# triSYCL/path_tracer

Measured on AMD Instinct MI355X. Metric: Msamples/s (W x H x spp / s) at 1080p 1024spp, higher is better.
Workload: dtype f32; 1 GPU; cornell: Cornell-style 7 box + 1 xy_rect + diffuse light, 1920x1080, 1024 spp, depth 50, seed = pixel linear id; hittables=8, mode=parity, frame_at_1_gpu=1920x1080

## Files before the change

path_tracer_amd/csrc/pt_device.hpp:

```cpp
#pragma once
#include <hip/hip_runtime.h>
#include <stdint.h>

#include "pt_math.hpp"

#ifdef PT_STAMPS
extern __device__ unsigned long long g_stamps[8];
#endif
#ifdef PT_STAMPS_TRI
extern __device__ unsigned long long g_tri[16];
#endif
#ifdef PT_STAMPS_RUNS
extern __device__ unsigned long long g_runs[16];
#endif
#ifdef PT_STAMPS_WALK
extern __device__ unsigned long long g_walk[8];
__device__ __forceinline__ unsigned long long* walk_ctr() { __shared__ unsigned long long c[8]; return c; }
#define PT_WALK_COUNT(i, v) do { const unsigned long long v_ = (unsigned long long)(v); if ((threadIdx.x & 63) == 0) atomicAdd(&walk_ctr()[i], v_); } while (0)
#else
#define PT_WALK_COUNT(i, v) do { } while (0)
#endif

namespace ptd {

// ... 820 lines not shown
  const cst_i4p lists = (cst_i4p)(cblob + lists_off);
  i4 cur = lists[0];
  for (int q = 0; q < q_static; ++q) {
    const i4 nxt = lists[q + 1];
    sphere_list_entry<false, K>(recs, cur, goff, 0.0f, c, h, accept_at);
    cur = nxt;
  }
  for (int q = 0; q < q_moving; ++q) {
    const i4 nxt = lists[q_static + q + 1];
    sphere_list_entry<true, K>(recs, cur, goff, frac, c, h, accept_at);
    cur = nxt;
  }
#ifdef PT_STAMPS_WALK
  const unsigned long long walk_t0 = __builtin_amdgcn_s_memtime();
  __builtin_amdgcn_sched_barrier(0);
#endif
  if constexpr (GRID == 1) { if (walk) sphere_grid_walk(recs, recs + w_cell, recs + w_cand, wg0, wg1, frac, goff, c, h, accept_at); }
  if constexpr (GRID == 2) {
    if (walk) {
      unsigned long long* slot;
      unsigned int* q;
      if constexpr (TRIPOOL) { slot = tri_slots() + (threadIdx.x & ~63); q = (unsigned int*)(tri_queue() + (threadIdx.x >> 6) * PT_TRI_QUEUE); }
      else { slot = sphere_slots() + (threadIdx.x & ~63); q = sphere_queue() + (threadIdx.x >> 6) * PT_SQ_CAP; }
      sphere_grid_walk_queued(recs, recs + w_cell, recs + w_cand, wg0, wg1, frac, (flags & 2) != 0, goff, c, h, slot, q, accept_at);
    }
  }
#ifdef PT_STAMPS_WALK
  asm volatile("" ::"v"(h.closest), "v"(h.hit));
  __builtin_amdgcn_sched_barrier(0);
  if (GRID && walk) { PT_WALK_COUNT(0, __builtin_amdgcn_s_memtime() - walk_t0); PT_WALK_COUNT(1, 1); }
#endif
}

template <bool FILTER, typename P>
__device__ __forceinline__ unsigned long long slab_chunk_pass(P xrecs, P slrecs, cst_f4p srecs, int cn, float bmax, const RayCtx& c, V3 om, V3 op, float& kdone,
                                                HitState& h) {
  const float none = as_f(PT_KEY_NONE);
  auto ku = [](float k) { return (unsigned int)as_i(k); };
  float k1 = none, k2 = none, k3 = none;
  typedef float f16v __attribute__((ext_vector_type(16)));
  typedef const __attribute__((address_space(4))) f16v* cst_f16p;
  const cst_f16p pairs = (cst_f16p)srecs;
  auto entry = [&](float lx, float ly, float lz, float hx, float hy, float hz, int j) {
    const float ax = __builtin_fmaf(lx, c.yx, om.x), bx = __builtin_fmaf(hx, c.yx, op.x);
    const float ay = __builtin_fmaf(ly, c.yy, om.y), by = __builtin_fmaf(hy, c.yy, op.y);
    const float az = __builtin_fmaf(lz, c.yz, om.z), bz = __builtin_fmaf(hz, c.yz, op.z);
    const float tn = __builtin_fmaxf(__builtin_fmaxf(__builtin_fminf(ax, bx), __builtin_fminf(ay, by)), __builtin_fminf(az, bz));
    const float tf = __builtin_fminf(__builtin_fminf(__builtin_fmaxf(ax, bx), __builtin_fmaxf(ay, by)), __builtin_fmaxf(az, bz));
    const float L = __builtin_fmaxf(tn, PT_TMIN);
    float key;
    asm("v_bfi_b32 %0, 15, %1, %2" : "=v"(key) : "s"(j), "v"(L));
    bool cand = L <= tf;
    if (FILTER) cand = cand & (ku(key) > ku(kdone));
    const float kk = cand ? key : none;
    asm("v_med3_u32 %0, %1, %0, %2" : "+v"(k3) : "v"(k2), "v"(kk));
    asm("v_med3_u32 %0, %1, %0, %2" : "+v"(k2) : "v"(k1), "v"(kk));
    asm("v_min_u32_e32 %0, %0, %1" : "+v"(k1) : "v"(kk));
  };
  for (int j = 0; j < cn; j += 2) {
    const f16v e = pairs[j >> 1];
    entry(e[0], e[1], e[2], e[4], e[5], e[6], j);
    entry(e[8], e[9], e[10], e[12], e[13], e[14], j + 1);
  }
  k1 = c.live ? k1 : none;
  k3 = c.live ? k3 : none;
  const unsigned long long had3 = __builtin_amdgcn_ballot_w64(ku(k3) != PT_KEY_NONE);
  unsigned long long vote;
#pragma unroll 1
  do {
    {
      bool inside = (ku(k1) ^ (unsigned int)as_i(PT_TMIN)) < 16u;
#ifdef PT_NO_POOL_PROOF
      inside = false;
#endif
      if (__builtin_amdgcn_ballot_w64(inside)) {
        const int offs = (as_i(k1) & 15) * 2;
        const f4 S0 = slrecs[offs], S1 = slrecs[offs + 1];
        const float e = 0x1p-20f, tlo = PT_TMIN * (1.0f - 0x1p-20f);
        auto ends = [&](float o, float y, float lo, float hi, float& lw, float& us, float& ws) {
          const float a = (lo - o) * y, b = (hi - o) * y;
          lw = __builtin_fminf(a, b);
          const float up = __builtin_fmaxf(a, b);
          const float S = __builtin_fmaf(__builtin_fabsf(o), 0x1.7p-21f, 0x1.dp-22f * bmax);
          const float w = __builtin_fmaf(__builtin_fabsf(y), S, up);
          us = __builtin_fmaf(__builtin_fabsf(up), -e, up);
          ws = __builtin_fmaf(__builtin_fabsf(w), e, w);
          return __builtin_fmaf(__builtin_fabsf(up), e, up) < PT_TMIN;
        };
        float lwx, lwy, lwz, usx, usy, usz, wsx, wsy, wsz;
        const bool ownx = ends(c.r.o.x, c.yx, S0.x, S1.x, lwx, usx, wsx);
        const bool owny = ends(c.r.o.y, c.yy, S0.y, S1.y, lwy, usy, wsy);
        const bool ownz = ends(c.r.o.z, c.yz, S0.z, S1.z, lwz, usz, wsz);
        const float lwm = __builtin_fmaxf(__builtin_fmaxf(lwx, lwy), lwz);
        const bool near_behind = __builtin_fmaf(__builtin_fabsf(lwm), e, lwm) < PT_TMIN;
        const bool kx = ownx & (usy > wsx) & (usz > wsx);
        const bool ky = owny & (usx > wsy) & (usz > wsy);
        const bool kz = ownz & (usx > wsz) & (usy > wsz);
        const bool gone = inside & near_behind & (kx | ky | kz);
        kdone = gone ? k1 : kdone;
        k1 = gone ? k2 : k1; k2 = gone ? k3 : k2; k3 = gone ? none : k3;
      }
    }
    asm("v_cmp_le_f32_e64 %0, %1, %2" : "=s"(vote) : "v"(as_i(k1) & ~15), "v"(h.closest));
    const bool active = __builtin_amdgcn_inverse_ballot_w64(vote);
#ifdef PT_STAMPS_POOL
    {
      const unsigned long long busy = __builtin_amdgcn_ballot_w64(active);
      if (vote != 0 && (threadIdx.x & 63) == 0) {
        atomicAdd(&g_stamps[5], 1ull);
        atomicAdd(&g_stamps[7], (unsigned long long)__builtin_popcountll(busy));
        if (FILTER) atomicAdd(&g_stamps[6], 1ull);
      }
    }
#endif
    if (active) {
      const int offl = (as_i(k1) & 15) * 2;
      const f4 X0 = xrecs[offl], X1 = xrecs[offl + 1];
      const unsigned long long exec_now = __builtin_amdgcn_ballot_w64(true);
      int hit_base = as_i(X0.w);
      const bool holder_later = ((h.hit >= 0) & (hit_off(h.hit) > hit_off(hit_base))) && hit_kind(h.hit) != DK_SPHERE;
      float cl = holder_later ? as_f(as_i(h.closest) - 1) : h.closest;
      int holder;
      asm("v_mov_b32_e32 %0, %1" : "=v"(holder) : "v"(h.hit));
      box_cmpx(X0, X1, c, exec_now, hit_base, cl, h.hit);
      asm("v_cmp_ne_u32_e32 vcc, %[hit], %[holder]\n\t"
          "v_mov_b32_e32 %[kd], %[k1]\n\t"
          "v_mov_b32_e32 %[k1], %[k2]\n\t"
          "v_cndmask_b32_e32 %[closest], %[closest], %[cl], vcc\n\t"
          "v_mov_b32_e32 %[k2], %[k3]\n\t"
          "v_mov_b32_e32 %[k3], %[none]"
          : [kd] "+v"(kdone), [k1] "+v"(k1), [k2] "+v"(k2), [k3] "+v"(k3), [closest] "+v"(h.closest)
          : [hit] "v"(h.hit), [holder] "v"(holder), [cl] "v"(cl), [none] "v"(none)
          : "vcc");
    }
  } while (vote != 0);
  return had3 & __builtin_amdgcn_ballot_w64(ku(k1) == PT_KEY_NONE);
}

template <typename P>
__device__ __forceinline__ void slab_pool(P blob, cst_f4p cblob, int pool_off, int n, float bmax, const RayCtx& c, HitState& h) {
  const float kP = 0x1.2p-21f;
  const float bP = 0x1.cp-22f * bmax;
  const V3 pp = mk(__builtin_fmaf(__builtin_fabsf(c.r.o.x), kP, bP), __builtin_fmaf(__builtin_fabsf(c.r.o.y), kP, bP),
                   __builtin_fmaf(__builtin_fabsf(c.r.o.z), kP, bP));
  const V3 yv = mk(c.yx, c.yy, c.yz);
  const V3 om = (mk(0.0f, 0.0f, 0.0f) - (c.r.o + pp)) * yv, op = (mk(0.0f, 0.0f, 0.0f) - (c.r.o - pp)) * yv;
#ifdef PT_STAMPS_POOL
  if ((threadIdx.x & 63) == 0) atomicAdd(&g_stamps[4], 1ull);
#endif
  for (int base = 0; base < n; base += 16) {
    const int cn = n - base < 16 ? n - base : 16;
    const P xrecs = blob + pool_off + 2 * (n + (n & 1)) + 2 * base;
    const cst_f4p srecs = cblob + pool_off + 2 * base;
    const P slrecs = blob + pool_off + 2 * base;
    float kdone = 0.0f;
    unsigned long long more = slab_chunk_pass<false>(xrecs, slrecs, srecs, cn, bmax, c, om, op, kdone, h);
    while (more) {
      if (!__builtin_amdgcn_inverse_ballot_w64(more)) kdone = as_f(PT_KEY_NONE);
      more = slab_chunk_pass<true>(xrecs, slrecs, srecs, cn, bmax, c, om, op, kdone, h);
    }
  }
}

#ifdef PT_STAMPS_TRI
#define PT_TRI_COUNT(i, v) do { const unsigned long long v_ = (unsigned long long)(v); if ((threadIdx.x & 63) == 0) atomicAdd(&g_tri[i], v_); } while (0)
#else
#define PT_TRI_COUNT(i, v) do { } while (0)
#endif
#define PT_TRI_WAVE_BITS(m) (__builtin_popcountll(__builtin_amdgcn_ballot_w64(((m) & 1u) != 0)) + __builtin_popcountll(__builtin_amdgcn_ballot_w64(((m) & 2u) != 0)) + \
                             __builtin_popcountll(__builtin_amdgcn_ballot_w64(((m) & 4u) != 0)) + __builtin_popcountll(__builtin_amdgcn_ballot_w64(((m) & 8u) != 0)))

__device__ __forceinline__ unsigned int gdword(glb_f4p pool, unsigned int base_f4, unsigned int i) { return ((const __attribute__((address_space(1))) unsigned int*)(pool + base_f4))[i]; }
__device__ __forceinline__ unsigned int gdword_stream(glb_f4p pool, unsigned int base_f4, unsigned int i) {
#ifdef PT_NT_LOADS
  return __builtin_nontemporal_load(((const __attribute__((address_space(1))) unsigned int*)(pool + base_f4)) + i);
#else
  return gdword(pool, base_f4, i);
#endif
}
__device__ __forceinline__ unsigned int sdword(glb_f4p pool, unsigned int base_f4, unsigned int i) {
  return ((const __attribute__((address_space(4))) unsigned int*)(unsigned long long)(pool + base_f4))[i];
}

typedef short short2_t __attribute__((ext_vector_type(2)));
#ifndef PT_BAND_PER
#define PT_BAND_PER 2
#endif
#define PT_TRI_BQUEUE (64 + 64 * PT_BAND_PER)
__device__ __forceinline__ f4* tri_bqueue() { __shared__ f4 s[4 * PT_TRI_BQUEUE]; return s; }
__device__ __forceinline__ int* tri_bqueue_idx() { __shared__ int s[4 * PT_TRI_BQUEUE]; return s; }
__device__ __forceinline__ unsigned long long tri_key(float t, int off) {
  return ((unsigned long long)(unsigned int)as_i(t) << 32) | (unsigned long long)(0xffffffffu - (unsigned int)off);
// ... 701 lines not shown
      if (IMG) { if (acc) { h.u = bu; h.v = bv; } }
    }
  }
}

__device__ __forceinline__ int record_size(int kind) {
  return kind == DK_SPHERE ? SZ_SPHERE : kind == DK_RECT ? SZ_RECT : (kind == DK_TRI || kind == DK_TRI_B) ? SZ_TRI : kind == DK_BOX ? SZ_BOX : SZ_MEDIUM;
}

template <bool IMG, bool BADOUEL = false, int GRID = 1, bool TRIPOOL = false, bool RECTBOX = false, bool DEFER = false, typename P>
__device__ __forceinline__ void hit_world_range(P blob, cst_f4p cblob, int ri0, int ri1, const RayCtx& c, bool fast, uint32_t& rng, HitState& h, const f4* pool = nullptr,
                                                TriDefer* dfr = nullptr, const TriPrimCtx* pc = nullptr) {
  for (int ri = ri0; ri < ri1; ++ri) {
#ifdef PT_STAMPS_RUNS
    const unsigned long long run_t0 = __builtin_amdgcn_s_memtime();
    __builtin_amdgcn_sched_barrier(0);
    struct RunStamp { unsigned long long t0; int ri; const HitState* h; __device__ ~RunStamp() { asm volatile("" ::"v"(h->closest), "v"(h->hit)); __builtin_amdgcn_sched_barrier(0);
      if ((threadIdx.x & 63) == 0) atomicAdd(&g_runs[ri < 15 ? ri : 15], __builtin_amdgcn_s_memtime() - t0); } } run_stamp{run_t0, ri, &h};
#endif
    f4 runf = cblob[ri];
    const int off = as_i(runf.y), kind = as_i(runf.x);
    if (!RECTBOX && (kind & DK_ABSORBED)) continue;
#ifdef PT_ABLATE_TAIL
    if (ri > 0) continue;
#endif
    if constexpr (RECTBOX) {
      static_assert(!IMG, "scenes of rects and boxes only have no image texture that tracks u, v");
      const f4 aux = cblob[off - 1];
      int span = fast ? as_i(aux.y) : 0;
#ifdef __HIP_DEVICE_COMPILE__
      asm volatile("" : "+s"(span));
#endif
      if (span != 0) {
        slab_pool(blob, cblob, as_i(aux.z), as_i(aux.w), aux.x, c, h);
        ri += span - 1;
      }
      hit_records_rectbox(blob + off, kind, span != 0 ? 0 : as_i(runf.z), off, c, fast, h);
    } else {
    if constexpr (!IMG) {
      if (fast && (kind == DK_RECT || kind == DK_BOX)) {
        const f4 aux = cblob[off - 1];
        if (as_i(aux.y) != 0) {
          slab_pool(blob, cblob, as_i(aux.z), as_i(aux.w), aux.x, c, h);
          ri += as_i(aux.y) - 1;
          continue;
        }
      }
    }
    hit_records<IMG, 1, 1, true, BADOUEL, GRID, TRIPOOL, RECTBOX, DEFER>(blob + off, cblob, kind, as_i(runf.z), off, c, fast, rng, h, (glb_f4p)pool, dfr, pc);
    }
  }
}
template <bool IMG, bool BADOUEL = false, int GRID = 1, bool TRIPOOL = false, bool RECTBOX = false, typename P>
__device__ __forceinline__ void hit_world(P blob, cst_f4p cblob, int n_runs, const RayCtx& c, bool fast, uint32_t& rng, HitState& h, const f4* pool = nullptr,
                                          const TriPrimCtx* pc = nullptr) {
  hit_begin(h);
  hit_world_range<IMG, BADOUEL, GRID, TRIPOOL, RECTBOX, false>(blob, cblob, 0, n_runs, c, fast, rng, h, pool, nullptr, pc);
}

__device__ __forceinline__ bool wave_all_regular(const RayCtx& c, bool live) {
  return __builtin_amdgcn_ballot_w64(live && !c.reg) == 0;
}

struct CoopScene {
  int n_runs;
  int coop_prefix;
};

__device__ __forceinline__ int nth_set_bit(unsigned long long m, int n) {
  for (int k = 0; k < n; ++k) m &= m - 1;
  return __builtin_ctzll(m);
}

__device__ __forceinline__ float shfl_f(float v, int src) { return __shfl(v, src, 64); }
__device__ __forceinline__ int shfl_i(int v, int src) { return __shfl(v, src, 64); }

// ... 360 lines not shown
```

path_tracer_amd/csrc/pt_flatten.hpp:

```cpp
#pragma once
#include <algorithm>
#include <cmath>
#include <cstdint>
#include <cstring>
#include <string>
#include <vector>

#include "../../include/pt_render.h"
#include "pt_tripool.hpp"

namespace ptf {

struct F4 {
  float x, y, z, w;
};
static_assert(sizeof(F4) == 16);

inline float as_f(int32_t i) { float f; std::memcpy(&f, &i, 4); return f; }

enum { DK_SPHERE = 0, DK_RECT = 1, DK_TRI = 2, DK_BOX = 3, DK_MEDIUM = 4, DK_TRI_B = 5 ,
       DK_ABSORBED = 8  };
enum { kHitOffBits = 25, kHitSideShift = 25, kHitKindShift = 28 };

struct PoolSegment { uint64_t at_f4; std::vector<uint32_t> dwords; };
struct PoolLayout {
  std::vector<PoolSegment> segments;
  uint64_t size_f4 = 0;
  uint32_t put(std::vector<uint32_t>&& v, int spare_f4) {
    const uint64_t at = size_f4;
    size_f4 += (v.size() + 3) / 4 + (uint64_t)spare_f4;
    segments.push_back(PoolSegment{at, std::move(v)});
    return (uint32_t)at;
  }
  void assemble(F4* out) const {
    std::memset((void*)out, 0, (size_t)size_f4 * 16);
    for (const PoolSegment& sg : segments) if (!sg.dwords.empty()) std::memcpy((void*)(out + sg.at_f4), sg.dwords.data(), sg.dwords.size() * 4);
  }
};
struct Flat {
  std::vector<F4> blob;
  std::vector<F4> mats;
  PoolLayout pool;
  int32_t n_runs = 0;
  bool has_image = false;
  bool has_medium = false;
  bool coop_ok = true;
  int32_t coop_prefix = 0;
  bool fast_ok = true;
  bool has_badouel = false;
  int grid_spheres = 0;
  int pooled = 0;
  int tri_pooled = 0;
  double tri_cells_per_triangle = 0;
  int tri_wide = 0, tri_maps = 0;
  long long tri_map_entries[3] = {0, 0, 0};
  int tri_map_res[3] = {0, 0, 0};
  int absorbed_spheres = 0;
  int tri_pool_runs = 0;
  int tri_pool_run = -1, tri_pool_hdr = 0, tri_pool_goff = 0, tri_pool_count = 0;
};

inline int device_kind(int32_t k) {
  switch (k) {
    case PT_HIT_SPHERE: return DK_SPHERE;
    case PT_HIT_XY_RECT: case PT_HIT_XZ_RECT: case PT_HIT_YZ_RECT: return DK_RECT;
    case PT_HIT_TRIANGLE: return DK_TRI;
    case PT_HIT_BOX: return DK_BOX;
    case PT_HIT_CONSTANT_MEDIUM: return DK_MEDIUM;
    default: return -1;
  }
}

inline int device_kind(const PtHittable& h) {
  if (h.kind == PT_HIT_TRIANGLE && h.strategy == PT_TRI_BADOUEL) return DK_TRI_B;
  return device_kind(h.kind);
}

inline int record_size(int dk) {
  switch (dk) { case DK_SPHERE: return 3; case DK_RECT: return 2; case DK_TRI: case DK_TRI_B: return 3; case DK_BOX: return 2; default: return 4; }
}

inline int validate(const PtSceneDesc* sc, std::string& err) {
  if (!sc) { err = "scene description is NULL"; return PT_ERR_INVALID_ARG; }
  if (sc->n_hittables < 0 || sc->n_materials < 0 || sc->n_textures < 0) { err = "negative table size"; return PT_ERR_INVALID_ARG; }
// ... 205 lines not shown
  for (uint32_t i : order) bandv.insert(bandv.end(), &tp.band_q[4 * (size_t)i], &tp.band_q[4 * (size_t)i] + 4);
  const uint32_t band = pool.put(std::move(bandv), 260);
  std::vector<uint32_t> readyv;
  readyv.reserve(12 * ntri);
  for (uint32_t i : order) for (int k = 0; k < 12; k++) readyv.push_back(bits(tp.band_ready[12 * (size_t)i + (size_t)k]));
  const uint32_t ready = pool.put(std::move(readyv), 192);
  const uint32_t cell_first = pool.put(std::move(tp.cell_first), 2);
  const uint32_t cell_cand = pool.put(std::move(tp.cell_cand), 20);
  uint32_t mfirst[kTriPoolMaxMaps] = {0, 0, 0}, mcand[kTriPoolMaxMaps] = {0, 0, 0};
  const int n_maps = std::min((int)tp.maps.size(), (int)kTriPoolMaxMaps);
  for (int k = 0; k < n_maps; k++) {
    TriDirMap& dm = tp.maps[(size_t)k];
    mfirst[k] = pool.put(std::move(dm.first), 2);
    mcand[k] = pool.put(std::move(dm.cand), 200);
  }
  const int32_t hdr = (int32_t)b.size();
  b.push_back({tp.origin[0], tp.origin[1], tp.origin[2], tp.inv_cell});
  b.push_back({as_f(tp.n[0]), as_f(tp.n[1]), as_f(tp.n[2]), tp.cell});
  b.push_back({tp.centre[0], tp.centre[1], tp.centre[2], tp.R});
  b.push_back({tp.rlimit2, tp.kappa, as_f((int32_t)ntri), as_f(n_maps)});
  b.push_back({as_f((int32_t)cell_first), as_f((int32_t)cell_cand), as_f((int32_t)tri_sorted), as_f((int32_t)band)});
  b.push_back({0.0f, tp.kq, tp.p_per_L, tp.kt});
  b.push_back({tp.ball_abs, tp.kr_a, tp.kr_b, tp.ea});
  b.push_back({tp.cq_lo[0], tp.cq_lo[1], tp.cq_lo[2], tp.eps_c});
  b.push_back({tp.cq_step[0], tp.cq_step[1], tp.cq_step[2], tp.eps_n});
  for (int k = 0; k < kTriPoolMaxMaps; k++) {
    if (k < n_maps) b.push_back({as_f(tp.maps[(size_t)k].R), tp.maps[(size_t)k].rho_max, as_f((int32_t)mfirst[k]), as_f((int32_t)mcand[k])});
    else b.push_back({as_f(0), -1.0f, as_f(0), as_f(0)});
  }
  b.push_back({as_f((int32_t)ready), 0.0f, 0.0f, 0.0f});
  return hdr;
}

inline int flatten(const PtSceneDesc* sc, Flat& out, std::string& err, bool allow_grid = true, int box_cull = 1, GridTuning tune = GridTuning(),
                   bool allow_tri_pool = true, TriPoolTuning tri_tune = TriPoolTuning(), bool sphere_merge = true) {
  int rc = validate(sc, err);
  if (rc) return rc;
  out = Flat();
  out.mats.reserve((size_t)sc->n_materials * 4);
  for (int i = 0; i < sc->n_materials; i++) {
    const PtMaterial& m = sc->materials[i];
    F4 M0{as_f(m.kind), as_f(PT_TEX_SOLID), m.param, 1.0f}, M1{m.color[0], m.color[1], m.color[2], as_f(1)},
        M2{0, 0, 0, as_f(1)}, M3{as_f(0), 0, 0, 0};
    if (m.kind == PT_MAT_LAMBERTIAN || m.kind == PT_MAT_LIGHTSOURCE || m.kind == PT_MAT_ISOTROPIC) {
      const PtTexture& t = sc->textures[m.texture];
      M0.y = as_f(t.kind);
      M0.w = t.freq;
      M1 = {t.color0[0], t.color0[1], t.color0[2], as_f((int32_t)t.width)};
      M2 = {t.color1[0], t.color1[1], t.color1[2], as_f((int32_t)t.height)};
      M3.x = as_f((int32_t)t.offset);
      if (t.kind == PT_TEX_IMAGE) out.has_image = true;
    }
    out.mats.push_back(M0); out.mats.push_back(M1); out.mats.push_back(M2); out.mats.push_back(M3);
  }
  struct Run { int kind, first, count; };
  std::vector<Run> runs;
  for (int i = 0; i < sc->n_hittables; i++) {
    int dk = device_kind(sc->hittables[i]);
    if (dk == DK_TRI_B) out.has_badouel = true;
    if (runs.empty() || runs.back().kind != dk) runs.push_back({dk, i, 0});
    runs.back().count++;
  }
  for (int i = 0; i < sc->n_hittables; i++) {
    const PtHittable& h = sc->hittables[i];
    bool rectish = h.kind == PT_HIT_XY_RECT || h.kind == PT_HIT_XZ_RECT || h.kind == PT_HIT_YZ_RECT || h.kind == PT_HIT_BOX ||
                   (h.kind == PT_HIT_CONSTANT_MEDIUM && h.boundary_kind == PT_HIT_BOX);
    if (!rectish) continue;
    int nf = (h.kind == PT_HIT_BOX || h.kind == PT_HIT_CONSTANT_MEDIUM) ? 6 : 5;
    for (int k = 0; k < nf; k++)
      if (!(std::fabs(h.f[k]) <= 1.152921504606846976e18f)) out.fast_ok = false;
    if (nf == 5) { if (!(h.f[0] <= h.f[1] && h.f[2] <= h.f[3])) out.fast_ok = false; }
// ... 46 lines not shown
  }
  struct Patch { size_t ri; std::vector<std::pair<size_t, size_t>> ranges; };
  std::vector<Patch> patches;
  for (size_t ri = 0; ri < runs.size(); ri++) {
    const Run& run = runs[ri];
    if (run.kind == DK_SPHERE) {
      std::vector<int32_t> codes;
      for (size_t k = 0; k < foreign_of[ri].size(); k++) codes.push_back(-(int32_t)(1 + k));
      Patch pt{ri, {}};
      out.grid_spheres += put_sphere_run_aux(b, &sc->hittables[run.first], run.count, allow_grid, tune, &codes, &pt.ranges);
      if (!codes.empty()) patches.push_back(std::move(pt));
      if (absorbed_by[ri] >= 0) { int32_t fl; std::memcpy(&fl, &b.back().w, 4); b.back().w = as_f(fl | 8); }
    }
    if (run.kind == DK_BOX || run.kind == DK_RECT) {
      const bool prev_rectish = ri > 0 && (runs[ri - 1].kind == DK_BOX || runs[ri - 1].kind == DK_RECT);
      int span = 0, n = 0, n_box = 0;
      if (!prev_rectish) {
        size_t rj = ri;
        while (rj < runs.size() && (runs[rj].kind == DK_BOX || runs[rj].kind == DK_RECT)) {
          n += runs[rj].count;
          if (runs[rj].kind == DK_BOX) n_box += runs[rj].count;
          rj++;
        }
        span = (int)(rj - ri);
      }
      const bool pool = box_cull && out.fast_ok && span > 0 && (box_cull == 2 ? n >= 2 : 88 * n_box - 7 * (n - n_box) > 200);
      float bmax = 0.0f;
      int32_t pool_off = 0;
      if (pool) {
        pool_off = (int32_t)b.size();
        pool_first = run.first;
        pool_at = b.size();
        const int ns = n + (n & 1);
        b.resize(b.size() + 2 * (size_t)ns + 2 * (size_t)n);
        pool_x = pool_at + 2 * (size_t)ns;
        if (ns > n) { const float q = std::nanf(""); b[pool_at + 2 * n] = {q, q, q, 0}; b[pool_at + 2 * n + 1] = {q, q, q, 0}; }
        const float ninf = -INFINITY;
        for (int e = 0; e < n; e++) {
          const PtHittable& h = sc->hittables[run.first + e];
          const float* f = h.f;
          F4 lo, hi, xhi;
          if (h.kind == PT_HIT_BOX) { lo = {f[0], f[1], f[2], 0}; hi = {f[3], f[4], f[5], 0}; xhi = hi; }
          else if (h.kind == PT_HIT_XY_RECT) { lo = {f[0], f[2], f[4], 0}; hi = {f[1], f[3], f[4], 0}; xhi = {f[1], f[3], ninf, 0}; }
          else if (h.kind == PT_HIT_XZ_RECT) { lo = {f[0], f[4], f[2], 0}; hi = {f[1], f[4], f[3], 0}; xhi = {f[1], ninf, f[3], 0}; }
          else { lo = {f[4], f[0], f[2], 0}; hi = {f[4], f[1], f[3], 0}; xhi = {ninf, f[1], f[3], 0}; }
          for (float v : {lo.x, lo.y, lo.z, hi.x, hi.y, hi.z}) bmax = std::max(bmax, std::fabs(v));
          b[pool_at + 2 * e] = lo; b[pool_at + 2 * e + 1] = hi;
          b[pool_x + 2 * e] = lo; b[pool_x + 2 * e + 1] = xhi;
        }
        pool_n = n;
        out.pooled += n;
      }
      b.push_back({bmax, as_f(pool ? span : 0), as_f(pool_off), as_f(pool ? n : 0)});
    }
    if (run.kind == DK_TRI) {
      int32_t hdr = 0;
      bool pooled = false;
      if (allow_tri_pool) {
        TriPool tp = build_tri_pool(&sc->hittables[run.first], run.count, tri_tune);
        unsigned long long map_f4 = 0;
        for (const TriDirMap& dm : tp.maps) { map_f4 += (dm.cand.size() + dm.first.size()) / 4 + 140; tri_tune.dm_budget -= (long long)dm.cand.size(); }
        tri_tune.dm_budget = std::max(0ll, tri_tune.dm_budget);
        if (tp.ok && out.pool.size_f4 + 12ull * (size_t)run.count + tp.cell_cand.size() / 4 + tp.cell_first.size() / 4 + map_f4 + 1024 < (1ull << 31)) {
          out.tri_cells_per_triangle = tp.mean_cells_per_triangle;
          out.tri_wide = tp.wide;
          out.tri_maps = (int)tp.maps.size();
          for (size_t k = 0; k < tp.maps.size() && k < 3; k++) { out.tri_map_entries[k] = (long long)tp.maps[k].cand.size(); out.tri_map_res[k] = tp.maps[k].R; }
          hdr = put_tri_pool(b, out.pool, tp, &sc->hittables[run.first], run.count);
          pooled = true;
          out.tri_pooled += run.count;
          out.tri_pool_runs++;
          out.tri_pool_run = (int)ri; out.tri_pool_hdr = hdr; out.tri_pool_goff = (int32_t)b.size() + 1; out.tri_pool_count = run.count;
        }
      }
      b.push_back({as_f(pooled ? 1 : 0), as_f(hdr), 0, 0});
    }
    b[ri] = {as_f(run.kind | (absorbed_by[ri] >= 0 ? DK_ABSORBED : 0)), as_f((int32_t)b.size()), as_f(run.count), as_f(run.first)};
    for (int i = run.first; i < run.first + run.count; i++) {
      const PtHittable& h = sc->hittables[i];
      const float* f = h.f;
      if (pool_n > 0 && i >= pool_first && i < pool_first + pool_n && (run.kind == DK_BOX || run.kind == DK_RECT))
// ... 16 lines not shown
          out.has_medium = true;
          int bk = h.boundary_kind == PT_HIT_SPHERE ? DK_SPHERE : DK_BOX;
          b.push_back({as_f(bk), f[9], as_f(h.material), as_f(i)});
          size_t before = b.size();
          if (bk == DK_SPHERE) put_sphere(b, f, h.material, i); else put_box(b, f, h.material, i);
          while (b.size() < before + 3) b.push_back({0, 0, 0, 0});
          break;
        }
      }
    }
  }
  for (const Patch& pt : patches) {
    int32_t base;
    std::memcpy(&base, &b[pt.ri].y, 4);
    for (const auto& rg : pt.ranges)
      for (size_t q = rg.first; q < rg.first + rg.second; q++) {
        float* w = &b[q].x;
        for (int j = 0; j < 4; j++) {
          int32_t v;
          std::memcpy(&v, &w[j], 4);
          if (v >= 0) continue;
          const Foreign& fo = foreign_of[pt.ri][(size_t)(-v - 1)];
          int32_t off_j;
          std::memcpy(&off_j, &b[(size_t)fo.run].y, 4);
          w[j] = as_f(off_j + 3 * fo.idx - base);
        }
      }
    out.absorbed_spheres += (int)foreign_of[pt.ri].size();
  }
  if (b.size() >= (1u << kHitOffBits)) { err = "scene too large for 25-bit record offsets (33.5 M records of 16 bytes)"; return PT_ERR_TOO_LARGE; }
  return PT_OK;
}

}
```

path_tracer_amd/csrc/pt_render.hip:

```cpp
#include <hip/hip_runtime.h>

#include <cmath>
#include <cstdio>
#include <cstdlib>
#include <cstring>
#include <map>
#include <memory>
#include <mutex>
#include <numeric>
#include <type_traits>
#include <string>
#include <vector>

#include "../../include/pt_render.h"
#include "pt_device.hpp"
#include "pt_flatten.hpp"

#ifdef PT_STAMPS
__device__ unsigned long long g_stamps[8];
#endif
#ifdef PT_STAMPS_WALK
__device__ unsigned long long g_walk[8];
#endif
#ifdef PT_STAMPS_RUNS
// ... 11 lines not shown
static_assert(sizeof(PtHittable) == 64 && sizeof(PtMaterial) == 32 && sizeof(PtTexture) == 48 && sizeof(PtCamera) == 96);
static_assert(sizeof(Cam) == sizeof(PtCamera));

namespace {

#ifndef PT_MIN_WAVES
#define PT_MIN_WAVES 7
#endif
#ifndef PT_MIN_WAVES_IMG
#define PT_MIN_WAVES_IMG 5
#endif
#ifndef PT_MIN_WAVES_CL
#define PT_MIN_WAVES_CL 7
#endif
#ifndef PT_MIN_WAVES_COOP
#define PT_MIN_WAVES_COOP 5
#endif
#ifndef PT_MIN_WAVES_TRIPOOL
#define PT_MIN_WAVES_TRIPOOL 5
#endif
#ifndef PT_MIN_WAVES_BINSTEP
#define PT_MIN_WAVES_BINSTEP 4
#endif
#ifndef PT_MIN_WAVES_COOP_IMG
#define PT_MIN_WAVES_COOP_IMG 5
#endif
enum { UV_NONE = 0, UV_WINNER = 1, UV_TRACKED = 2 };
constexpr int kBlock = 256;
constexpr int kWavesPerBlock = kBlock / 64;
#ifndef PT_GRID_BLOCK
#define PT_GRID_BLOCK 256
#endif
constexpr int kGridBlock = PT_GRID_BLOCK;
constexpr size_t kMaxLdsBlob = 64 * 1024;
constexpr size_t kMaxLdsWithMaterials = 16 * 1024;
constexpr size_t kMaxLdsColdScene = 10 * 1024;
constexpr float kCoopMinTraversal = 2500.0f;
constexpr int kGridMinTiles = 0;
constexpr unsigned kQueueRing = 256;

struct KArgs {
  Cam cam = {};
  const f4* blob = nullptr;
  const f4* mats = nullptr;
  const f4* pool = nullptr;
  const uint8_t* atlas = nullptr;
  float* fb = nullptr;
  int n_runs = 0, blob_f4 = 0, mats_f4 = 0;
  int width = 0, height = 0, samples = 0, depth = 0;
  float inv_w = 0.0f, inv_h = 0.0f;
  int pinhole = 0;
  int shard_index = 0, shard_count = 0;
  int tiles_x = 0, n_tiles = 0;
  int n_local_pixels = 0;
  unsigned int* queue = nullptr;
  unsigned int* cost = nullptr;
  unsigned int* resume_rng = nullptr;
  int resume_spp = 0;
  int keep_state = 0;
  const uint8_t* mask = nullptr;
  int prio_onset = 0, prio_t1 = 0, prio_t2 = 0, prio_t3 = 0;
  int cost_max = 0;
  const int* order = nullptr;
  const int* n_split = nullptr;
  int tile_granular = 0;
  int tile_group = 64;
  int heavy_pixels = 0;
// ... 924 lines not shown
  if (const char* e = std::getenv("PT_GRID_WALK")) t.grid_walk = std::atoi(e);
  if (const char* e = std::getenv("PT_LANES_CAP")) t.lanes_cap = std::atoi(e) <= 0 ? -1 : std::min(64, std::atoi(e));
  if (const char* e = std::getenv("PT_HEAVY_TILES")) t.heavy_tiles = std::atoi(e) <= 0 ? -1 : std::atoi(e);
}
static int resolve_tuning(const PtTuning* user, PtTuning& t, std::string& err) {
  if (!user) { tuning_env(t); return PT_OK; }
  if (user->struct_size < 8 || user->struct_size > (int32_t)sizeof(PtTuning)) { err = "PtTuning.struct_size is not a size this library knows (use pt_tuning_init)"; return PT_ERR_INVALID_ARG; }
  tuning_defaults(t);
  std::memcpy(&t, user, (size_t)user->struct_size);
  t.struct_size = (int32_t)sizeof(PtTuning);
  return PT_OK;
}

static int flatten_tuned(const PtSceneDesc* desc, const PtTuning& t, ptf::Flat& flat, std::string& err) {
  const int box_cull = t.slab_pools < 0 ? 0 : t.slab_pools > 0 ? 2 : 1;
  ptf::GridTuning tune;
  if (t.grid_margin > 0.0f) tune.m = t.grid_margin;
  if (t.grid_cell > 0.0f) tune.cell = t.grid_cell;
  const bool allow_grid = t.sphere_grid >= 0;
  bool allow_tri = t.tri_pool >= 0;
  for (int i = 0; desc && desc->hittables && i < desc->n_hittables && allow_tri; i++)
    if (desc->hittables[i].kind == PT_HIT_TRIANGLE && desc->hittables[i].strategy == PT_TRI_BADOUEL) allow_tri = false;
  ptf::TriPoolTuning tri;
  if (t.tri_min_run > 0) tri.min_run = t.tri_min_run;
  if (t.tri_M > 0.0f) tri.M = t.tri_M;
  for (int k = 0; k < 3; k++) if (t.tri_res[k] > 0) tri.dm_res[k] = t.tri_res[k];
  if (t.tri_rho[0] != 0.0f) tri.dm_rho[0] = t.tri_rho[0];
  if (t.tri_rho[1] != 0.0f) tri.dm_rho[1] = t.tri_rho[1];
  if (t.tri_rho2 != 0.0f) tri.dm_rho[2] = t.tri_rho2;
  if (t.tri_budget_mb > 0) tri.dm_budget = (long long)t.tri_budget_mb * (1 << 18);
  if (t.tri_cell > 0.0f) tri.cell = t.tri_cell;
  if (const char* e = std::getenv("PT_TRI_GRID_BUDGET")) tri.grid_budget = (float)std::atof(e);
  const bool merge = t.sphere_merge >= 0;
  int rc = ptf::flatten(desc, flat, err, allow_grid, box_cull, tune, allow_tri, tri, merge);
  if (rc) return rc;
  if (flat.grid_spheres > 0 && flat.blob.size() * 16 > kMaxLdsBlob) {
    ptf::Flat plain;
    std::string err2;
    if (flat.tri_pooled == 0 && ptf::flatten(desc, plain, err2, false, box_cull, tune, allow_tri, tri, merge) == PT_OK && plain.blob.size() * 16 <= kMaxLdsBlob) flat = std::move(plain);
  }
  return PT_OK;
}

int fail(int code, const std::string& msg) {
  g_last_error = msg;
  return code;
}

#define PT_HIP(expr)                                                                             \
  do {                                                                                           \
    hipError_t e_ = (expr);                                                                      \
    if (e_ != hipSuccess) return fail(PT_ERR_HIP, std::string(#expr) + ": " + hipGetErrorString(e_)); \
  } while (0)

struct Knobs {
  int blocks_per_cu = 0;
  bool no_cold_lds = false;
  int wide_logG = 0;
  bool has_split_tiles = false;
  int split_tiles = 0;
  int lpt_max = -1, probe_spp_max = 16;
  int grid_min_tiles = kGridMinTiles;
  float model_fixed = 2400.0f, model_chain = 2400.0f;
  int scatter_log = 0;
  bool lpt_with_scatter = false;
  bool no_scatter = false;
  bool generic_materials = false;
  int grid_walk = 0;
  int lanes_cap = 0;
  bool no_tri_cache = false;
  bool no_chain_prio = false;
  bool no_resume = false;
// ... 36 lines not shown
  ~DevBuf() { if (p) (void)hipFree(p); }
  hipError_t alloc(size_t n) {
    if (p) (void)hipFree(p);
    p = nullptr; cap = 0;
    const hipError_t e = hipMalloc((void**)&p, std::max<size_t>(n, 1) * sizeof(T));
    if (e == hipSuccess) cap = n; else p = nullptr;
    return e;
  }
  hipError_t grow(size_t n) { return p && cap >= n ? hipSuccess : alloc(n); }
};

}

struct PtScene {
  DevBuf<f4> blob;
  f4* mats = nullptr;
  DevBuf<f4> pool;
  size_t pool_bytes = 0;
  DevBuf<uint8_t> atlas;
  int n_runs = 0, blob_f4 = 0, mats_f4 = 0;
  bool has_image = false;
  bool track_uv = false;
  bool fast_ok = false;
  bool coop_ok = false;
  bool has_badouel = false;
  int coop_prefix = 0;
  int n_hittables = 0;
  mutable bool last_had_wide_phase = false;
  mutable int last_launch[4] = {0, 0, 0, 0};
  mutable int nsplit_override = 0;
  float traversal_cost = 0.0f;
  int grid_spheres = 0;
  int tri_pooled = 0;
  bool rectbox_only = false;
  bool mats_simple = false;
  size_t blob_bytes = 0, atlas_bytes = 0;
  int num_cus = 256;
  size_t lds_per_block = 64 * 1024;
  mutable DevBuf<unsigned int> ws_cost;
  mutable DevBuf<unsigned int> ws_rank;
  mutable DevBuf<unsigned int> ws_rng;
  mutable DevBuf<int> ws_order;
  DevBuf<int> ws_nsplit;
  mutable DevBuf<float> ws_partial;
  int bin_run = -1, bin_hdr = 0, bin_goff = 0, bin_keys = 0, bin_full_slices = 1, bin_base1 = 0;
  bool binned = false;
  mutable DevBuf<unsigned int> ws_tricache;
  mutable DevBuf<char> ws_bin;
  mutable int last_generations = 0;
  DevBuf<unsigned int> queues;
  mutable unsigned int next_queue = 0;
  mutable hipEvent_t ring_done[kQueueRing] = {};
  int device = 0;
  mutable std::mutex sched;
  mutable std::map<const void*, int> occupancy;
  Knobs knobs;
};

namespace {


struct KV {
  int uv = UV_NONE;
  bool lds = false, mlds = false, coop = false, cl = false, fast = false, badouel = false;
  int grid = 1;
  bool tripool = false;
// ... 26 lines not shown

template <int MATS>
Kernel headline_kernel(bool lds, bool mlds, bool cold) {
  if (!lds) return kernel_of<KV{.grid = 0, .mats = MATS}>;
  if (cold) return kernel_of<KV{.lds = true, .mlds = true, .cl = true, .grid = 0, .mats = MATS}>;
  return mlds ? kernel_of<KV{.lds = true, .mlds = true, .grid = 0, .mats = MATS}> : kernel_of<KV{.lds = true, .grid = 0, .mats = MATS}>;
}

struct BinKernels { void (*step)(BinArgs); void (*finish)(BinArgs); };
template <int UV, int MATS>
constexpr BinKernels bin_kernels = {bin_step_kernel<UV, MATS>, bin_finish_kernel<UV, MATS>};

struct Variant {
  int rc = PT_OK;
  Kernel kernel = nullptr;
  size_t shmem = 0;
  int coop_prefix = -1;
  bool tri_pool = false;
  bool resident = false;
  bool use_grid = false;
  bool coop = false;
  bool chain_bound = false;
  bool queued_walk = false;
};

template <int UV>
Variant choose_variant_uv(const PtScene* s, const PtRenderParams* p, int local_tiles, bool fast, int n_local_pixels) {
  Variant v;
  const bool fast_ok = s->fast_ok && !(p->flags & PT_FLAG_NO_FASTDIV);
  v.coop_prefix = (s->coop_ok && fast_ok && !(p->flags & PT_FLAG_NO_COOP)) ? s->coop_prefix : -1;
  const size_t blob_bytes = (size_t)s->blob_f4 * 16;
  v.tri_pool = s->tri_pooled > 0 && !(p->flags & PT_FLAG_FORCE_STREAM);
  v.resident = (blob_bytes <= kMaxLdsBlob || (p->flags & PT_FLAG_NO_LDS) || v.tri_pool) && !(p->flags & PT_FLAG_FORCE_STREAM);
  const bool lds = v.resident && !(p->flags & PT_FLAG_NO_LDS) && !v.tri_pool;
  const bool mlds = lds && blob_bytes + (size_t)s->mats_f4 * 16 <= kMaxLdsWithMaterials;
  v.shmem = lds ? blob_bytes + (mlds ? (size_t)s->mats_f4 * 16 : 0) : 0;
  const bool cold = mlds && v.shmem <= kMaxLdsColdScene && !s->knobs.no_cold_lds;
  v.use_grid = s->grid_spheres > 0 && v.resident  && local_tiles >= s->knobs.grid_min_tiles && !(p->flags & PT_FLAG_FORCE_COOP);
  v.coop = lds && v.coop_prefix >= 0 && !v.use_grid && (s->traversal_cost >= kCoopMinTraversal || (p->flags & PT_FLAG_FORCE_COOP));

  if (s->has_badouel) {
    if (fast) { v.rc = fail(PT_ERR_INVALID_ARG, "PT_FLAG_FAST_RNG is not offered for scenes with Badouel-strategy triangles"); return v; }
    v.kernel = !v.resident ? render_kernel_stream<UV, false, true> : kernel_of<KV{.uv = UV, .badouel = true}>;
    return v;
  }
  if (fast) {
    if (v.tri_pool) v.kernel = tripool_kernel(UV, true);
    else if (!v.resident) v.kernel = render_kernel_stream<UV, true>;
    else if (!lds) v.kernel = kernel_of<KV{.uv = UV, .fast = true}>;
    else v.kernel = mlds ? kernel_of<KV{.uv = UV, .lds = true, .mlds = true, .fast = true}> : kernel_of<KV{.uv = UV, .lds = true, .fast = true}>;
    return v;
  }
  if (v.tri_pool) { v.kernel = tripool_kernel(UV, false); return v; }
  if (!v.resident) { v.kernel = render_kernel_stream<UV>; return v; }
  if constexpr (UV == UV_NONE) {
    if (s->grid_spheres == 0 && !v.coop) {
      v.chain_bound = true;
      v.kernel = !s->mats_simple    ? headline_kernel<MATS_ALL>(lds, mlds, cold)
                 : !s->rectbox_only ? headline_kernel<MATS_LAMB_LIGHT_SOLID>(lds, mlds, cold)
                                    : headline_kernel<MATS_LAMB_LIGHT_SOLID | MATS_RECTBOX_ONLY>(lds, mlds, cold);
      return v;
    }
  }
  if (!lds) { v.kernel = kernel_of<KV{.uv = UV}>; return v; }
  if (v.coop) { v.kernel = mlds ? kernel_of<KV{.uv = UV, .lds = true, .mlds = true, .coop = true}> : kernel_of<KV{.uv = UV, .lds = true, .coop = true}>; return v; }
  if constexpr (UV == UV_NONE) {
    if (cold) { v.kernel = kernel_of<KV{.lds = true, .mlds = true, .cl = true}>; return v; }
// ... 162 lines not shown
  if (rc) return fail(rc, err);
  lap("flatten (+ culling tables)");
  int ndev = 0;
  if (hipGetDeviceCount(&ndev) != hipSuccess || ndev == 0) return fail(PT_ERR_NO_DEVICE, "no HIP device visible");
  std::unique_ptr<PtScene> owner(new PtScene());
  PtScene* const s = owner.get();
  s->knobs = Knobs(tun);
  PT_HIP(hipGetDevice(&s->device));
  {
    hipDeviceProp_t prop;
    PT_HIP(hipGetDeviceProperties(&prop, s->device));
    s->num_cus = prop.multiProcessorCount;
    s->lds_per_block = prop.sharedMemPerBlock;
  }
  s->n_runs = flat.n_runs;
  s->blob_f4 = (int)flat.blob.size();
  s->has_image = flat.has_image;
  s->fast_ok = flat.fast_ok;
  s->coop_ok = flat.coop_ok && !flat.has_badouel;
  s->has_badouel = flat.has_badouel;
  s->track_uv = flat.has_image && !flat.coop_ok;
  s->coop_prefix = flat.coop_prefix;
  s->n_hittables = desc->n_hittables;
  for (int i = 0; i < desc->n_hittables; i++) {
    switch (desc->hittables[i].kind) {
      case PT_HIT_SPHERE: s->traversal_cost += 22.0f; break;
      case PT_HIT_TRIANGLE: s->traversal_cost += 35.0f; break;
      case PT_HIT_BOX: s->traversal_cost += 120.0f; break;
      case PT_HIT_CONSTANT_MEDIUM: s->traversal_cost += 300.0f; break;
      default: s->traversal_cost += 20.0f; break;
    }
  }
  s->grid_spheres = flat.grid_spheres;
  s->rectbox_only = desc->n_hittables > 0 && !s->knobs.generic_materials;
#ifdef PT_NO_RECTBOX
  s->rectbox_only = false;
#endif
  for (int i = 0; i < desc->n_hittables && s->rectbox_only; i++) {
    const int k = desc->hittables[i].kind;
    if (k != PT_HIT_XY_RECT && k != PT_HIT_XZ_RECT && k != PT_HIT_YZ_RECT && k != PT_HIT_BOX) s->rectbox_only = false;
  }
  s->mats_simple = desc->n_materials > 0 && !s->knobs.generic_materials;
  for (int i = 0; i < desc->n_materials && s->mats_simple; i++) {
    const PtMaterial& m = desc->materials[i];
    if ((m.kind != PT_MAT_LAMBERTIAN && m.kind != PT_MAT_LIGHTSOURCE) || desc->textures[m.texture].kind != PT_TEX_SOLID) s->mats_simple = false;
  }
  s->tri_pooled = flat.has_badouel ? 0 : flat.tri_pooled;
  if (s->tri_pooled > 0 && flat.tri_pool_runs == 1 && !s->track_uv && tun.tri_binned > 0) {
    s->binned = true;
    s->bin_run = flat.tri_pool_run; s->bin_hdr = flat.tri_pool_hdr; s->bin_goff = flat.tri_pool_goff;
    s->bin_full_slices = std::min(64, std::max(1, (flat.tri_pool_count + 2047) / 2048));
    long long keys = 2;
    for (int k = 0; k < flat.tri_maps && k < 3; k++) keys += 3ll * flat.tri_map_res[k] * flat.tri_map_res[k];
    s->bin_keys = (int)keys;
    s->bin_base1 = flat.tri_maps > 0 ? 3 * flat.tri_map_res[0] * flat.tri_map_res[0] : 0;
  }
  s->blob_bytes = flat.blob.size() * 16;
  s->mats_f4 = (int)flat.mats.size();
  const size_t blob_bytes = flat.blob.size() * 16, mats_bytes = flat.mats.size() * 16;
  PT_HIP(s->blob.alloc(flat.blob.size() + flat.mats.size()));
  s->mats = s->blob.p + flat.blob.size();
  if (blob_bytes) PT_HIP(hipMemcpy(s->blob.p, flat.blob.data(), blob_bytes, hipMemcpyHostToDevice));
  if (mats_bytes) PT_HIP(hipMemcpy(s->mats, flat.mats.data(), mats_bytes, hipMemcpyHostToDevice));
  if (flat.pool.size_f4) {
    s->pool_bytes = (size_t)flat.pool.size_f4 * 16;
    PT_HIP(s->pool.alloc((size_t)flat.pool.size_f4));
// ... 1057 lines not shown
```

Baseline: 17760 Msamples/s.

## Precompute per-octant near/far box corners for LDS slab pool tests

Adds a per-box table of 8 ray-direction-octant corner pairs to the pooled box records, so the LDS slab test can load near/far corners directly and skip the per-axis min/max. The ray's octant picks the table offset, which roughly halves the ALU work of each box test at the cost of extra LDS footprint and an LDS-address gather per entry. The layout falls back to the old format if the blob would exceed the LDS limit, and pools without octant tables are no longer allowed in LDS. For the Cornell boxes (a pooled run) this path is likely taken.

```diff
diff --git a/path_tracer_amd/csrc/pt_device.hpp b/path_tracer_amd/csrc/pt_device.hpp
--- a/path_tracer_amd/csrc/pt_device.hpp
+++ b/path_tracer_amd/csrc/pt_device.hpp
@@ -876,12 +876,45 @@
 #endif
 }
 
-template <bool FILTER, typename P>
-__device__ __forceinline__ unsigned long long slab_chunk_pass(P xrecs, P slrecs, cst_f4p srecs, int cn, float bmax, const RayCtx& c, V3 om, V3 op, float& kdone,
+template <bool FILTER, int FORM, typename P>
+__device__ __forceinline__ unsigned long long slab_chunk_pass(P xrecs, P slrecs, cst_f4p srecs, P otab, int cn, float bmax, const RayCtx& c, V3 om, V3 op, float& kdone,
                                                 HitState& h) {
+  constexpr bool OCT = FORM > 0;
   const float none = as_f(PT_KEY_NONE);
   auto ku = [](float k) { return (unsigned int)as_i(k); };
   float k1 = none, k2 = none, k3 = none;
+  auto insert = [&](float L, float tf, int j) {
+    float key;
+    asm("v_bfi_b32 %0, 15, %1, %2" : "=v"(key) : "s"(j), "v"(L));
+    bool cand = L <= tf;
+    if (FILTER) cand = cand & (ku(key) > ku(kdone));
+    const float kk = cand ? key : none;
+    asm("v_med3_u32 %0, %1, %0, %2" : "+v"(k3) : "v"(k2), "v"(kk));
+    asm("v_med3_u32 %0, %1, %0, %2" : "+v"(k2) : "v"(k1), "v"(kk));
+    asm("v_min_u32_e32 %0, %0, %1" : "+v"(k1) : "v"(kk));
+  };
+  if constexpr (OCT) {
+    auto entry = [&](f4 N, f4 F, int j) {
+      const float nx = __builtin_fmaf(N.x, c.yx, om.x), ny = __builtin_fmaf(N.y, c.yy, om.y), nz = __builtin_fmaf(N.z, c.yz, om.z);
+      const float fx = __builtin_fmaf(F.x, c.yx, op.x), fy = __builtin_fmaf(F.y, c.yy, op.y), fz = __builtin_fmaf(F.z, c.yz, op.z);
+      const float L = __builtin_fmaxf(__builtin_fmaxf(__builtin_fmaxf(nx, ny), nz), PT_TMIN);
+      insert(L, __builtin_fminf(__builtin_fminf(fx, fy), fz), j);
+    };
+#pragma unroll 1
+    for (int j = 0; j < cn; j += FORM) {
+      unsigned int at;
+      asm("v_lshl_add_u32 %0, %1, 8, %2" : "=v"(at) : "s"(j), "v"((unsigned int)(uintptr_t)otab));
+      const P e = (P)(uintptr_t)at;
+      if constexpr (FORM == 2) {
+        const f4 N0 = e[0], F0 = e[1], N1 = e[16], F1 = e[17];
+        entry(N0, F0, j);
+        entry(N1, F1, j + 1);
+      } else {
+        const f4 N0 = e[0], F0 = e[1];
+        entry(N0, F0, j);
+      }
+    }
+  } else {
   typedef float f16v __attribute__((ext_vector_type(16)));
   typedef const __attribute__((address_space(4))) f16v* cst_f16p;
   const cst_f16p pairs = (cst_f16p)srecs;
@@ -891,20 +924,13 @@
     const float az = __builtin_fmaf(lz, c.yz, om.z), bz = __builtin_fmaf(hz, c.yz, op.z);
     const float tn = __builtin_fmaxf(__builtin_fmaxf(__builtin_fminf(ax, bx), __builtin_fminf(ay, by)), __builtin_fminf(az, bz));
     const float tf = __builtin_fminf(__builtin_fminf(__builtin_fmaxf(ax, bx), __builtin_fmaxf(ay, by)), __builtin_fmaxf(az, bz));
-    const float L = __builtin_fmaxf(tn, PT_TMIN);
-    float key;
-    asm("v_bfi_b32 %0, 15, %1, %2" : "=v"(key) : "s"(j), "v"(L));
-    bool cand = L <= tf;
-    if (FILTER) cand = cand & (ku(key) > ku(kdone));
-    const float kk = cand ? key : none;
-    asm("v_med3_u32 %0, %1, %0, %2" : "+v"(k3) : "v"(k2), "v"(kk));
-    asm("v_med3_u32 %0, %1, %0, %2" : "+v"(k2) : "v"(k1), "v"(kk));
-    asm("v_min_u32_e32 %0, %0, %1" : "+v"(k1) : "v"(kk));
+    insert(__builtin_fmaxf(tn, PT_TMIN), tf, j);
   };
   for (int j = 0; j < cn; j += 2) {
     const f16v e = pairs[j >> 1];
     entry(e[0], e[1], e[2], e[4], e[5], e[6], j);
     entry(e[8], e[9], e[10], e[12], e[13], e[14], j + 1);
+  }
   }
   k1 = c.live ? k1 : none;
   k3 = c.live ? k3 : none;
@@ -918,13 +944,20 @@
       inside = false;
 #endif
       if (__builtin_amdgcn_ballot_w64(inside)) {
-        const int offs = (as_i(k1) & 15) * 2;
-        const f4 S0 = slrecs[offs], S1 = slrecs[offs + 1];
+        f4 S0, S1;
+        if constexpr (OCT) {
+          unsigned int at;
+          asm("v_lshl_add_u32 %0, %1, 8, %2" : "=v"(at) : "v"(as_i(k1) & 15), "v"((unsigned int)(uintptr_t)otab));
+          S0 = ((P)(uintptr_t)at)[0]; S1 = ((P)(uintptr_t)at)[1];
+        } else {
+          const int offs = (as_i(k1) & 15) * 2;
+          S0 = slrecs[offs]; S1 = slrecs[offs + 1];
+        }
         const float e = 0x1p-20f, tlo = PT_TMIN * (1.0f - 0x1p-20f);
         auto ends = [&](float o, float y, float lo, float hi, float& lw, float& us, float& ws) {
           const float a = (lo - o) * y, b = (hi - o) * y;
-          lw = __builtin_fminf(a, b);
-          const float up = __builtin_fmaxf(a, b);
+          lw = OCT ? a : __builtin_fminf(a, b);
+          const float up = OCT ? b : __builtin_fmaxf(a, b);
           const float S = __builtin_fmaf(__builtin_fabsf(o), 0x1.7p-21f, 0x1.dp-22f * bmax);
           const float w = __builtin_fmaf(__builtin_fabsf(y), S, up);
           us = __builtin_fmaf(__builtin_fabsf(up), -e, up);
@@ -981,14 +1014,28 @@
   return had3 & __builtin_amdgcn_ballot_w64(ku(k1) == PT_KEY_NONE);
 }
 
-template <typename P>
+template <int LDS_FORM, typename P>
 __device__ __forceinline__ void slab_pool(P blob, cst_f4p cblob, int pool_off, int n, float bmax, const RayCtx& c, HitState& h) {
+  constexpr int FORM = __is_same(P, lds_f4p) ? LDS_FORM : 0;
+  constexpr bool OCT = FORM > 0;
   const float kP = 0x1.2p-21f;
   const float bP = 0x1.cp-22f * bmax;
   const V3 pp = mk(__builtin_fmaf(__builtin_fabsf(c.r.o.x), kP, bP), __builtin_fmaf(__builtin_fabsf(c.r.o.y), kP, bP),
                    __builtin_fmaf(__builtin_fabsf(c.r.o.z), kP, bP));
   const V3 yv = mk(c.yx, c.yy, c.yz);
-  const V3 om = (mk(0.0f, 0.0f, 0.0f) - (c.r.o + pp)) * yv, op = (mk(0.0f, 0.0f, 0.0f) - (c.r.o - pp)) * yv;
+  V3 om, op;
+  P otab = blob;
+  if constexpr (OCT) {
+    const V3 ps = mk(__builtin_copysignf(pp.x, c.yx), __builtin_copysignf(pp.y, c.yy), __builtin_copysignf(pp.z, c.yz));
+    const V3 ny = mk(-c.yx, -c.yy, -c.yz);
+    om = (c.r.o + ps) * ny;
+    op = (c.r.o - ps) * ny;
+    const unsigned int q2 = (((unsigned int)as_i(c.yx) >> 30) & 2u) | (((unsigned int)as_i(c.yy) >> 29) & 4u) | (((unsigned int)as_i(c.yz) >> 28) & 8u);
+    otab = blob + pool_off + 2 * (n + (n & 1)) + 2 * n + (int)q2;
+  } else {
+    om = (mk(0.0f, 0.0f, 0.0f) - (c.r.o + pp)) * yv;
+    op = (mk(0.0f, 0.0f, 0.0f) - (c.r.o - pp)) * yv;
+  }
 #ifdef PT_STAMPS_POOL
   if ((threadIdx.x & 63) == 0) atomicAdd(&g_stamps[4], 1ull);
 #endif
@@ -997,11 +1044,12 @@
     const P xrecs = blob + pool_off + 2 * (n + (n & 1)) + 2 * base;
     const cst_f4p srecs = cblob + pool_off + 2 * base;
     const P slrecs = blob + pool_off + 2 * base;
+    const P ochunk = otab + 16 * base;
     float kdone = 0.0f;
-    unsigned long long more = slab_chunk_pass<false>(xrecs, slrecs, srecs, cn, bmax, c, om, op, kdone, h);
+    unsigned long long more = slab_chunk_pass<false, FORM>(xrecs, slrecs, srecs, ochunk, cn, bmax, c, om, op, kdone, h);
     while (more) {
       if (!__builtin_amdgcn_inverse_ballot_w64(more)) kdone = as_f(PT_KEY_NONE);
-      more = slab_chunk_pass<true>(xrecs, slrecs, srecs, cn, bmax, c, om, op, kdone, h);
+      more = slab_chunk_pass<true, FORM>(xrecs, slrecs, srecs, ochunk, cn, bmax, c, om, op, kdone, h);
     }
   }
 }
@@ -1769,7 +1817,7 @@
       asm volatile("" : "+s"(span));
 #endif
       if (span != 0) {
-        slab_pool(blob, cblob, as_i(aux.z), as_i(aux.w), aux.x, c, h);
+        slab_pool<2>(blob, cblob, as_i(aux.z), as_i(aux.w), aux.x, c, h);
         ri += span - 1;
       }
       hit_records_rectbox(blob + off, kind, span != 0 ? 0 : as_i(runf.z), off, c, fast, h);
@@ -1778,7 +1826,7 @@
       if (fast && (kind == DK_RECT || kind == DK_BOX)) {
         const f4 aux = cblob[off - 1];
         if (as_i(aux.y) != 0) {
-          slab_pool(blob, cblob, as_i(aux.z), as_i(aux.w), aux.x, c, h);
+          slab_pool<GRID == 2 ? 0 : 1>(blob, cblob, as_i(aux.z), as_i(aux.w), aux.x, c, h);
           ri += as_i(aux.y) - 1;
           continue;
         }
diff --git a/path_tracer_amd/csrc/pt_flatten.hpp b/path_tracer_amd/csrc/pt_flatten.hpp
--- a/path_tracer_amd/csrc/pt_flatten.hpp
+++ b/path_tracer_amd/csrc/pt_flatten.hpp
@@ -50,6 +50,7 @@
   bool has_badouel = false;
   int grid_spheres = 0;
   int pooled = 0;
+  bool pool_octants = false;
   int tri_pooled = 0;
   double tri_cells_per_triangle = 0;
   int tri_wide = 0, tri_maps = 0;
@@ -321,11 +322,12 @@
   return hdr;
 }
 
-inline int flatten(const PtSceneDesc* sc, Flat& out, std::string& err, bool allow_grid = true, int box_cull = 1, GridTuning tune = GridTuning(),
-                   bool allow_tri_pool = true, TriPoolTuning tri_tune = TriPoolTuning(), bool sphere_merge = true) {
+inline int flatten_layout(const PtSceneDesc* sc, Flat& out, std::string& err, bool allow_grid, int box_cull, GridTuning tune,
+                          bool allow_tri_pool, TriPoolTuning tri_tune, bool sphere_merge, bool pool_octants) {
   int rc = validate(sc, err);
   if (rc) return rc;
   out = Flat();
+  out.pool_octants = pool_octants;
   out.mats.reserve((size_t)sc->n_materials * 4);
   for (int i = 0; i < sc->n_materials; i++) {
     const PtMaterial& m = sc->materials[i];
@@ -438,7 +440,7 @@
         pool_first = run.first;
         pool_at = b.size();
         const int ns = n + (n & 1);
-        b.resize(b.size() + 2 * (size_t)ns + 2 * (size_t)n);
+        b.resize(b.size() + 2 * (size_t)ns + 2 * (size_t)n + (pool_octants ? 16 * (size_t)ns : 0));
         pool_x = pool_at + 2 * (size_t)ns;
         if (ns > n) { const float q = std::nanf(""); b[pool_at + 2 * n] = {q, q, q, 0}; b[pool_at + 2 * n + 1] = {q, q, q, 0}; }
         const float ninf = -INFINITY;
@@ -453,6 +455,17 @@
           for (float v : {lo.x, lo.y, lo.z, hi.x, hi.y, hi.z}) bmax = std::max(bmax, std::fabs(v));
           b[pool_at + 2 * e] = lo; b[pool_at + 2 * e + 1] = hi;
           b[pool_x + 2 * e] = lo; b[pool_x + 2 * e + 1] = xhi;
+        }
+        if (pool_octants) {
+          const size_t oct = pool_x + 2 * (size_t)n;
+          for (int e = 0; e < ns; e++) {
+            const F4 lo = b[pool_at + 2 * e], hi = b[pool_at + 2 * e + 1];
+            for (int q = 0; q < 8; q++) {
+              const bool sx = q & 1, sy = q & 2, sz = q & 4;
+              b[oct + 16 * (size_t)e + 2 * q] = {sx ? hi.x : lo.x, sy ? hi.y : lo.y, sz ? hi.z : lo.z, 0};
+              b[oct + 16 * (size_t)e + 2 * q + 1] = {sx ? lo.x : hi.x, sy ? lo.y : hi.y, sz ? lo.z : hi.z, 0};
+            }
+          }
         }
         pool_n = n;
         out.pooled += n;
@@ -535,4 +548,16 @@
   return PT_OK;
 }
 
-}
+constexpr size_t kLdsImageBytes = 64 * 1024;
+inline int flatten(const PtSceneDesc* sc, Flat& out, std::string& err, bool allow_grid = true, int box_cull = 1, GridTuning tune = GridTuning(),
+                   bool allow_tri_pool = true, TriPoolTuning tri_tune = TriPoolTuning(), bool sphere_merge = true, bool pool_octants = true) {
+  size_t records_f4 = 0;
+  for (int i = 0; sc && sc->hittables && i < sc->n_hittables; i++) records_f4 += (size_t)std::max(0, record_size(device_kind(sc->hittables[i])));
+  const bool with_tables = pool_octants && records_f4 * 16 <= kLdsImageBytes;
+  int rc = flatten_layout(sc, out, err, allow_grid, box_cull, tune, allow_tri_pool, tri_tune, sphere_merge, with_tables);
+  if (rc == PT_OK && with_tables && out.pooled > 0 && out.blob.size() * 16 > kLdsImageBytes)
+    rc = flatten_layout(sc, out, err, allow_grid, box_cull, tune, allow_tri_pool, tri_tune, sphere_merge, false);
+  return rc;
+}
+
+}
diff --git a/path_tracer_amd/csrc/pt_render.hip b/path_tracer_amd/csrc/pt_render.hip
--- a/path_tracer_amd/csrc/pt_render.hip
+++ b/path_tracer_amd/csrc/pt_render.hip
@@ -67,7 +67,7 @@
 #define PT_GRID_BLOCK 256
 #endif
 constexpr int kGridBlock = PT_GRID_BLOCK;
-constexpr size_t kMaxLdsBlob = 64 * 1024;
+constexpr size_t kMaxLdsBlob = ptf::kLdsImageBytes;
 constexpr size_t kMaxLdsWithMaterials = 16 * 1024;
 constexpr size_t kMaxLdsColdScene = 10 * 1024;
 constexpr float kCoopMinTraversal = 2500.0f;
@@ -1058,12 +1058,13 @@
   if (t.tri_cell > 0.0f) tri.cell = t.tri_cell;
   if (const char* e = std::getenv("PT_TRI_GRID_BUDGET")) tri.grid_budget = (float)std::atof(e);
   const bool merge = t.sphere_merge >= 0;
-  int rc = ptf::flatten(desc, flat, err, allow_grid, box_cull, tune, allow_tri, tri, merge);
+  const bool octants = !std::getenv("PT_NO_POOL_OCTANTS");
+  int rc = ptf::flatten(desc, flat, err, allow_grid, box_cull, tune, allow_tri, tri, merge, octants);
   if (rc) return rc;
   if (flat.grid_spheres > 0 && flat.blob.size() * 16 > kMaxLdsBlob) {
     ptf::Flat plain;
     std::string err2;
-    if (flat.tri_pooled == 0 && ptf::flatten(desc, plain, err2, false, box_cull, tune, allow_tri, tri, merge) == PT_OK && plain.blob.size() * 16 <= kMaxLdsBlob) flat = std::move(plain);
+    if (flat.tri_pooled == 0 && ptf::flatten(desc, plain, err2, false, box_cull, tune, allow_tri, tri, merge, octants) == PT_OK && plain.blob.size() * 16 <= kMaxLdsBlob) flat = std::move(plain);
   }
   return PT_OK;
 }
@@ -1166,6 +1167,7 @@
   float traversal_cost = 0.0f;
   int grid_spheres = 0;
   int tri_pooled = 0;
+  bool pools_need_scalar = false;
   bool rectbox_only = false;
   bool mats_simple = false;
   size_t blob_bytes = 0, atlas_bytes = 0;
@@ -1258,7 +1260,7 @@
   const size_t blob_bytes = (size_t)s->blob_f4 * 16;
   v.tri_pool = s->tri_pooled > 0 && !(p->flags & PT_FLAG_FORCE_STREAM);
   v.resident = (blob_bytes <= kMaxLdsBlob || (p->flags & PT_FLAG_NO_LDS) || v.tri_pool) && !(p->flags & PT_FLAG_FORCE_STREAM);
-  const bool lds = v.resident && !(p->flags & PT_FLAG_NO_LDS) && !v.tri_pool;
+  const bool lds = v.resident && !(p->flags & PT_FLAG_NO_LDS) && !v.tri_pool && !s->pools_need_scalar;
   const bool mlds = lds && blob_bytes + (size_t)s->mats_f4 * 16 <= kMaxLdsWithMaterials;
   v.shmem = lds ? blob_bytes + (mlds ? (size_t)s->mats_f4 * 16 : 0) : 0;
   const bool cold = mlds && v.shmem <= kMaxLdsColdScene && !s->knobs.no_cold_lds;
@@ -1487,6 +1489,7 @@
     }
   }
   s->grid_spheres = flat.grid_spheres;
+  s->pools_need_scalar = flat.pooled > 0 && !flat.pool_octants;
   s->rectbox_only = desc->n_hittables > 0 && !s->knobs.generic_materials;
 #ifdef PT_NO_RECTBOX
   s->rectbox_only = false;
```

After: 19540 Msamples/s, median of 6. 10.0% higher.
